# Elody-07/AWR-Adaptive-Weighting-Regression

Hardware: AMD Instinct MI355X
Metric: depth-images/sec (train step) (higher is better)
Workload: dtype f32; 1 GPU; resnet_18-deconv NYU-shape 128x128 J=14 train step (GT-map+fwd+head+Huber+bwd+Adam), batch 64/GPU = BASELINE configs[1]; global_batch=64, img_size=128, joints=14, parallelism=dp1, hipgraph=False, wgrad_streams=2, independent_hw_queues_for_side_streams=3, gemm_products=1, deterministic=False, device_cus=256, nhwc_head_loss=True, launcher=direct

## Files before the change

### awr-adaptive-weighting-regression_amd/csrc/awr_elem.hip

```cpp
#include <math.h>

#include <stdlib.h>

#include "awr_common.h"

namespace awr {

__global__ __launch_bounds__(256) void pack_weight_kernel(const float* __restrict__ w, int d0, int d1, int T, int transpose, int n_pad,
                                                          int ld, float* __restrict__ out) {
    const int64_t total = (int64_t)n_pad * T * ld;
    const int64_t idx = (int64_t)blockIdx.x * 256 + threadIdx.x;
    if (idx >= total) return;
    const int c = (int)(idx % ld);
    const int t = (int)((idx / ld) % T);
    const int n = (int)(idx / ((int64_t)ld * T));
    float v = 0.f;
    if (!transpose) {
        if (n < d0 && c < d1) v = w[((int64_t)n * d1 + c) * T + t];
    } else {
        if (n < d1 && c < d0) v = w[((int64_t)c * d1 + n) * T + t];
    }
    out[idx] = v;
}

__global__ __launch_bounds__(256) void unpack_wgrad_kernel(const float* __restrict__ packed, int d0, int d1, int T, int ld,
                                                           float* __restrict__ grad, int accumulate) {
    const int64_t total = (int64_t)d0 * d1 * T;
    const int64_t idx = (int64_t)blockIdx.x * 256 + threadIdx.x;
    if (idx >= total) return;
    const int t = (int)(idx % T);
    const int b = (int)((idx / T) % d1);
    const int a = (int)(idx / ((int64_t)T * d1));
    const float v = packed[((int64_t)a * T + t) * ld + b];
    grad[idx] = accumulate ? grad[idx] + v : v;
}

template <typename Job>
__device__ __forceinline__ int find_job(const Job* __restrict__ jobs, int n, int64_t idx) {
    int lo = 0, hi = n - 1;
    while (lo < hi) {
        const int mid = (lo + hi + 1) >> 1;
        if (jobs[mid].first <= idx) lo = mid; else hi = mid - 1;
    }
    return lo;
}

__device__ __forceinline__ void store_split_elem(void* split, int64_t idx, float x) {
    const unsigned h = __float_as_uint(x) & 0xFFFF0000u;
    const float r1 = x - __uint_as_float(h);
    const unsigned m = __float_as_uint(r1) & 0xFFFF0000u;
    const unsigned l = __float_as_uint(r1 - __uint_as_float(m));
    unsigned short* o = reinterpret_cast<unsigned short*>(split) + (idx >> 5) * 96 + (idx & 31);
    o[0] = (unsigned short)(h >> 16);
    o[32] = (unsigned short)(m >> 16);
    o[64] = (unsigned short)(l >> 16);
}

constexpr int PACK_TILE = 8192;

__global__ __launch_bounds__(256) void pack_batched_kernel(const awr_pack_job* __restrict__ jobs, int n) {
    __shared__ float tile[PACK_TILE + 64];
    const awr_pack_job jb = jobs[find_job(jobs, n, (int64_t)blockIdx.x)];
    const int r = (int)((int64_t)blockIdx.x - jb.first);
    const int T = jb.T, TS = T | 1, ld = jb.ld;
    const int inner = jb.transpose ? jb.d0 : jb.d1, valid_rows = jb.transpose ? jb.d1 : jb.d0;
    const bool rok = r < valid_rows;
    const int cch = (PACK_TILE / TS) & ~31;
    const int cols = jb.cols > 0 ? jb.cols : ld;
    for (int c0 = 0; c0 < cols; c0 += cch) {
        const int cc = cols - c0 < cch ? cols - c0 : cch;
        for (int i = threadIdx.x; i < cc * T; i += 256) {
            const int c = i / T, t = i - c * T;
            float v = 0.f;
            if (rok && c0 + c < inner)
                v = jb.transpose ? jb.src[((int64_t)(c0 + c) * jb.d1 + r) * T + t] : jb.src[((int64_t)r * jb.d1 + c0 + c) * T + t];
            tile[c * TS + t] = v;
        }
        __syncthreads();
        for (int i = threadIdx.x; i < cc * T; i += 256) {
            const int t = i / cc, c = i - t * cc;
            const float v = tile[c * TS + t];
            const int64_t o = ((int64_t)r * T + t) * ld + c0 + c;
            jb.dst[o] = v;
            if (jb.split) store_split_elem(jb.split, o, v);
        }
        __syncthreads();
    }
}

__global__ __launch_bounds__(256) void split_weight_kernel(const float* __restrict__ packed, void* __restrict__ split, int64_t n) {
    const int64_t idx = (int64_t)blockIdx.x * 256 + threadIdx.x;
    if (idx < n) store_split_elem(split, idx, packed[idx]);
}

__global__ __launch_bounds__(256) void unpack_batched_kernel(const awr_unpack_job* __restrict__ jobs, int n) {
    __shared__ float tile[PACK_TILE + 64];
    const awr_unpack_job jb = jobs[find_job(jobs, n, (int64_t)blockIdx.x)];
    const int a = (int)((int64_t)blockIdx.x - jb.first);
    const int T = jb.T, TS = T | 1, d1 = jb.d1;
    const int cch = (PACK_TILE / TS) & ~31;
    for (int c0 = 0; c0 < d1; c0 += cch) {
        const int cc = d1 - c0 < cch ? d1 - c0 : cch;
        for (int i = threadIdx.x; i < cc * T; i += 256) {
            const int t = i / cc, c = i - t * cc;
            const float* src = jb.packed + ((int64_t)a * T + t) * jb.ld + c0 + c;
            float v = src[0];
            for (int k = 1; k < jb.slots; ++k) v += src[(int64_t)k * jb.slot_stride];
            tile[c * TS + t] = v;
        }
        __syncthreads();
        for (int i = threadIdx.x; i < cc * T; i += 256) {
            const int c = i / T, t = i - c * T;
            jb.grad[((int64_t)a * d1 + c0 + c) * T + t] = tile[c * TS + t];
        }
        __syncthreads();
    }
}

__global__ __launch_bounds__(256) void stem_im2col_kernel(const float* __restrict__ img, int B, int H, int W, float* __restrict__ cols) {
    const int64_t idx = (int64_t)blockIdx.x * 256 + threadIdx.x;
    const int64_t total = (int64_t)B * H * W * 8;
    if (idx >= total) return;
    const int k0 = (int)(idx & 7) * 4;
    const int64_t pix = idx >> 3;
    const int x = (int)(pix % W), y = (int)((pix / W) % H);
    const int64_t b = pix / ((int64_t)W * H);
    float v[4];
#pragma unroll
    for (int i = 0; i < 4; ++i) {
        const int k = k0 + i;
        const int yy = y + k / 5 - 2, xx = x + k % 5 - 2;
        v[i] = (k < 25 && yy >= 0 && yy < H && xx >= 0 && xx < W) ? img[(b * H + yy) * W + xx] : 0.f;
    }
    st4(cols + idx * 4, make_float4(v[0], v[1], v[2], v[3]));
}

__global__ __launch_bounds__(64) void bn_finalize_kernel(double* __restrict__ stats, int C, int nslots, double count, const float* __restrict__ gamma,
                                   const float* __restrict__ beta, float* __restrict__ rmean, float* __restrict__ rvar, float momentum,
                                   float eps, float* __restrict__ scale, float* __restrict__ shift, float* __restrict__ mean_o,
                                   float* __restrict__ invstd_o) {
    const int c = blockIdx.x;
    double s1 = 0.0, s2 = 0.0;
    for (int k = threadIdx.x; k < nslots; k += 64) {
        s1 += stats[(size_t)k * 2 * C + c];
        s2 += stats[(size_t)k * 2 * C + C + c];
        stats[(size_t)k * 2 * C + c] = 0.0;
        stats[(size_t)k * 2 * C + C + c] = 0.0;
    }
    s1 = wave_sum(s1);
    s2 = wave_sum(s2);
    if (threadIdx.x != 0) return;
    const double mean = s1 / count;
    double var = s2 / count - mean * mean;
    if (var < 0.0) var = 0.0;
    const float invstd = (float)(1.0 / sqrt(var + (double)eps));
    const float g = gamma ? gamma[c] : 1.f, b = beta ? beta[c] : 0.f;
    const float sc = g * invstd;
    scale[c] = sc;
    shift[c] = b - (float)mean * sc;
    if (mean_o) mean_o[c] = (float)mean;
    if (invstd_o) invstd_o[c] = invstd;
    if (rmean) rmean[c] = (1.f - momentum) * rmean[c] + momentum * (float)mean;
    if (rvar) {
        const double unb = count > 1.0 ? var * count / (count - 1.0) : var;
        rvar[c] = (1.f - momentum) * rvar[c] + momentum * (float)unb;
    }
}

__global__ void bn_fold_eval_kernel(int C, const float* __restrict__ gamma, const float* __restrict__ beta, const float* __restrict__ rmean,
                                    const float* __restrict__ rvar, float eps, float* __restrict__ scale, float* __restrict__ shift) {
    const int c = blockIdx.x * blockDim.x + threadIdx.x;
    if (c >= C) return;
    const float sc = gamma[c] / sqrtf(rvar[c] + eps);
    scale[c] = sc;
    shift[c] = beta[c] - rmean[c] * sc;
}

struct prod_geom { int H, W, k, s, p, Ho, Wo, in_relu; };
template <int MODE>
__global__ __launch_bounds__(256) void col_reduce_kernel(const float* __restrict__ x, const float* __restrict__ act, const float* __restrict__ y,
                                                         const float* __restrict__ mean, const float* __restrict__ invstd,
                                                         const float* __restrict__ msc, const float* __restrict__ msh, int64_t npix,
                                                         int C, int Cw, int rows_per_block, int nslots, double* __restrict__ out64, float* __restrict__ out32,
                                                         prod_geom pg = prod_geom(), float* __restrict__ pout = nullptr, uint8_t* __restrict__ parg = nullptr) {
    const int cb = blockIdx.y * Cw;
    if (Cw > C - cb) Cw = C - cb;
    const int C4 = Cw >> 2;
    const int rpp = 256 / C4;
    const int cg = threadIdx.x % C4, rg = threadIdx.x / C4;
    const bool active = rg < rpp;
    const int64_t r0 = (int64_t)blockIdx.x * rows_per_block;
    int64_t r1 = r0 + rows_per_block;
    if (r1 > npix) r1 = npix;
    float4 s1 = make_float4(0, 0, 0, 0), s2 = make_float4(0, 0, 0, 0);
    float4 mu = make_float4(0, 0, 0, 0), is = make_float4(1, 1, 1, 1);
    float4 ks = make_float4(0, 0, 0, 0), kt = make_float4(0, 0, 0, 0);
    if (MODE == 1 && active) {
        mu = ld4(mean + cb + cg * 4);
        is = ld4(invstd + cb + cg * 4);
        if (msc) {
            ks = ld4(msc + cb + cg * 4);
            kt = ld4(msh + cb + cg * 4);
        }
    }
    float4 c0 = make_float4(0, 0, 0, 0);
    int nrows = 0;
    if (MODE == 0 && active && r0 + rg < r1) c0 = ld4(x + (r0 + rg) * C + cb + cg * 4);
    auto accum = [&](float4 v, float4 aa, float4 yy) {
        if (MODE == 0) {
            v.x -= c0.x; v.y -= c0.y; v.z -= c0.z; v.w -= c0.w;
            s1.x += v.x; s1.y += v.y; s1.z += v.z; s1.w += v.w;
            s2.x += v.x * v.x; s2.y += v.y * v.y; s2.z += v.z * v.z; s2.w += v.w * v.w;
            ++nrows;
        } else if (MODE == 1) {
            if (act) {
                v.x = aa.x > 0.f ? v.x : 0.f; v.y = aa.y > 0.f ? v.y : 0.f; v.z = aa.z > 0.f ? v.z : 0.f; v.w = aa.w > 0.f ? v.w : 0.f;
            } else if (msc) {
                v.x = yy.x * ks.x + kt.x > 0.f ? v.x : 0.f; v.y = yy.y * ks.y + kt.y > 0.f ? v.y : 0.f;
                v.z = yy.z * ks.z + kt.z > 0.f ? v.z : 0.f; v.w = yy.w * ks.w + kt.w > 0.f ? v.w : 0.f;
            }
            s1.x += v.x; s1.y += v.y; s1.z += v.z; s1.w += v.w;
            s2.x += v.x * ((yy.x - mu.x) * is.x); s2.y += v.y * ((yy.y - mu.y) * is.y);
            s2.z += v.z * ((yy.z - mu.z) * is.z); s2.w += v.w * ((yy.w - mu.w) * is.w);
        } else {
            s1.x += v.x; s1.y += v.y; s1.z += v.z; s1.w += v.w;
        }
    };
    if (MODE >= 3 && active) {
        bool first = true;
        float4 ks4 = make_float4(1, 1, 1, 1), kt4 = make_float4(0, 0, 0, 0);
        if (MODE == 3 && msc) { ks4 = ld4(msc + cb + cg * 4); kt4 = ld4(msh + cb + cg * 4); }
        auto consume = [&](int64_t r, float4 v) {
            st4(pout + r * C + cb + cg * 4, v);
            if (first) { c0 = v; first = false; }
            v.x -= c0.x; v.y -= c0.y; v.z -= c0.z; v.w -= c0.w;
            s1.x += v.x; s1.y += v.y; s1.z += v.z; s1.w += v.w;
            s2.x += v.x * v.x; s2.y += v.y * v.y; s2.z += v.z * v.z; s2.w += v.w * v.w;
            ++nrows;
        };
        int64_t r = r0 + rg;
        constexpr int U = 4;
        if (MODE == 4 || (pg.k == 2 && pg.s == 2 && pg.p == 0)) {
            for (; r + (int64_t)(U - 1) * rpp < r1; r += (int64_t)U * rpp) {
                float4 w[U][4];
                int64_t rr[U];
#pragma unroll
                for (int u = 0; u < U; ++u) {
                    rr[u] = r + (int64_t)u * rpp;
                    const int ox = (int)(rr[u] % pg.Wo), oy = (int)((rr[u] / pg.Wo) % pg.Ho);
                    const int64_t b = rr[u] / ((int64_t)pg.Wo * pg.Ho);
                    if (MODE == 4) {
                        w[u][0] = ld4(x + rr[u] * C + cb + cg * 4);
                        w[u][1] = ld4(act + ((b * pg.H + (oy >> 1)) * pg.W + (ox >> 1)) * C + cb + cg * 4);
                    } else {
                        const float* base = x + ((b * pg.H + 2 * oy) * pg.W + 2 * ox) * C + cb + cg * 4;
                        w[u][0] = ld4(base); w[u][1] = ld4(base + C); w[u][2] = ld4(base + (int64_t)pg.W * C); w[u][3] = ld4(base + (int64_t)pg.W * C + C);
                    }
                }
#pragma unroll
                for (int u = 0; u < U; ++u) {
                    if (MODE == 4) {
                        consume(rr[u], make_float4(w[u][0].x + w[u][1].x, w[u][0].y + w[u][1].y, w[u][0].z + w[u][1].z, w[u][0].w + w[u][1].w));
                    } else {
                        float m[4] = {-INFINITY, -INFINITY, -INFINITY, -INFINITY};
                        int am[4] = {0, 0, 0, 0};
#pragma unroll
                        for (int t = 0; t < 4; ++t) {
                            float4 q = w[u][t];
                            if (msc) {
                                q.x = q.x * ks4.x + kt4.x; q.y = q.y * ks4.y + kt4.y; q.z = q.z * ks4.z + kt4.z; q.w = q.w * ks4.w + kt4.w;
                                if (pg.in_relu) { q.x = fmaxf(q.x, 0.f); q.y = fmaxf(q.y, 0.f); q.z = fmaxf(q.z, 0.f); q.w = fmaxf(q.w, 0.f); }
                            }
                            const float qq[4] = {q.x, q.y, q.z, q.w};
#pragma unroll
                            for (int c = 0; c < 4; ++c)
                                if (qq[c] > m[c]) { m[c] = qq[c]; am[c] = t; }
                        }
                        if (parg) *reinterpret_cast<uchar4*>(parg + rr[u] * C + cb + cg * 4) = make_uchar4((uint8_t)am[0], (uint8_t)am[1], (uint8_t)am[2], (uint8_t)am[3]);
                        consume(rr[u], make_float4(m[0], m[1], m[2], m[3]));
                    }
                }
            }
        }
        for (; r < r1; r += rpp) {
            const int ox = (int)(r % pg.Wo), oy = (int)((r / pg.Wo) % pg.Ho);
            const int64_t b = r / ((int64_t)pg.Wo * pg.Ho);
            float4 v;
            if (MODE == 3) {
                float m[4] = {-INFINITY, -INFINITY, -INFINITY, -INFINITY};
                int am[4] = {0, 0, 0, 0};
                for (int ky = 0; ky < pg.k; ++ky) {
                    const int yy = oy * pg.s - pg.p + ky;
                    if (yy < 0 || yy >= pg.H) continue;
                    for (int kx = 0; kx < pg.k; ++kx) {
                        const int xx = ox * pg.s - pg.p + kx;
                        if (xx < 0 || xx >= pg.W) continue;
                        float4 w = ld4(x + ((b * pg.H + yy) * pg.W + xx) * C + cb + cg * 4);
                        if (msc) {
                            w.x = w.x * ks4.x + kt4.x; w.y = w.y * ks4.y + kt4.y; w.z = w.z * ks4.z + kt4.z; w.w = w.w * ks4.w + kt4.w;
                            if (pg.in_relu) { w.x = fmaxf(w.x, 0.f); w.y = fmaxf(w.y, 0.f); w.z = fmaxf(w.z, 0.f); w.w = fmaxf(w.w, 0.f); }
                        }
                        const float ww[4] = {w.x, w.y, w.z, w.w};
#pragma unroll
                        for (int c = 0; c < 4; ++c)
                            if (ww[c] > m[c]) { m[c] = ww[c]; am[c] = ky * pg.k + kx; }
                    }
                }
                v = make_float4(m[0], m[1], m[2], m[3]);
                if (parg) *reinterpret_cast<uchar4*>(parg + r * C + cb + cg * 4) = make_uchar4((uint8_t)am[0], (uint8_t)am[1], (uint8_t)am[2], (uint8_t)am[3]);
            } else {
                const float4 u = ld4(x + r * C + cb + cg * 4), l = ld4(act + ((b * pg.H + (oy >> 1)) * pg.W + (ox >> 1)) * C + cb + cg * 4);
                v = make_float4(u.x + l.x, u.y + l.y, u.z + l.z, u.w + l.w);
            }
            consume(r, v);
        }
    } else if (active) {
        constexpr int U = 4;
        int64_t r = r0 + rg;
        const float4 z4 = make_float4(0, 0, 0, 0);
        for (; r + (int64_t)(U - 1) * rpp < r1; r += (int64_t)U * rpp) {
            float4 v[U], aa[U], yy[U];
#pragma unroll
            for (int u = 0; u < U; ++u) {
                const int64_t o = (r + (int64_t)u * rpp) * C + cb + cg * 4;
                v[u] = ld4(x + o);
                aa[u] = (MODE == 1 && act) ? ld4(act + o) : z4;
                yy[u] = (MODE == 1) ? ld4(y + o) : z4;
            }
#pragma unroll
            for (int u = 0; u < U; ++u) accum(v[u], aa[u], yy[u]);
        }
        for (; r < r1; r += rpp) {
            const int64_t o = r * C + cb + cg * 4;
            accum(ld4(x + o), (MODE == 1 && act) ? ld4(act + o) : z4, (MODE == 1) ? ld4(y + o) : z4);
        }
    }
    __shared__ double sh1[256][4], sh2[256][4];
    {
        const float p[4] = {s1.x, s1.y, s1.z, s1.w}, q[4] = {s2.x, s2.y, s2.z, s2.w}, c[4] = {c0.x, c0.y, c0.z, c0.w};
#pragma unroll
        for (int k = 0; k < 4; ++k) {
            const double cc = (double)c[k], n = (double)nrows;
            sh1[threadIdx.x][k] = (double)p[k] + n * cc;
            sh2[threadIdx.x][k] = (double)q[k] + 2.0 * cc * (double)p[k] + n * cc * cc;
        }
    }
    __syncthreads();
    if (threadIdx.x < C4) {
        double a[4] = {0, 0, 0, 0}, b[4] = {0, 0, 0, 0};
        for (int g = 0; g < rpp; ++g) {
#pragma unroll
            for (int k = 0; k < 4; ++k) {
                a[k] += sh1[g * C4 + threadIdx.x][k];
                b[k] += sh2[g * C4 + threadIdx.x][k];
            }
        }
#pragma unroll
        for (int k = 0; k < 4; ++k) {
            const int c = cb + threadIdx.x * 4 + k;
            if (MODE == 2) {
                atomicAdd(out32 + c, (float)a[k]);
            } else {
                double* o = out64 + (size_t)(blockIdx.x % nslots) * 2 * C;
                atomicAdd(o + c, a[k]);
                atomicAdd(o + C + c, b[k]);
            }
        }
    }
}

__global__ __launch_bounds__(256) void bn_apply_kernel(const float* __restrict__ x, const float* __restrict__ scale, const float* __restrict__ shift,
                                                       const float* __restrict__ res, int relu, float* __restrict__ out, int64_t n4, int C4) {
    const int64_t i = (int64_t)blockIdx.x * 256 + threadIdx.x;
    if (i >= n4) return;
    const int cg = (int)(i % C4);
    const float4 v = ld4(x + i * 4), sc = ld4(scale + cg * 4), sh = ld4(shift + cg * 4);
    float4 o = make_float4(v.x * sc.x + sh.x, v.y * sc.y + sh.y, v.z * sc.z + sh.z, v.w * sc.w + sh.w);
    if (res) {
        const float4 r = ld4(res + i * 4);
        o.x += r.x; o.y += r.y; o.z += r.z; o.w += r.w;
    }
    if (relu) {
        o.x = fmaxf(o.x, 0.f); o.y = fmaxf(o.y, 0.f); o.z = fmaxf(o.z, 0.f); o.w = fmaxf(o.w, 0.f);
    }
    st4(out + i * 4, o);
}

__global__ __launch_bounds__(64) void bn_bwd_finalize_kernel(double* __restrict__ sums, int C, int nslots, double inv_count, const float* __restrict__ gamma,
                                       const float* __restrict__ invstd, float* __restrict__ coef, float* __restrict__ dgamma,
                                       float* __restrict__ dbeta, int accumulate, const float* __restrict__ mean = nullptr, float* __restrict__ lin = nullptr) {
    const int c = blockIdx.x;
    double s1 = 0.0, s2 = 0.0;
    for (int k = threadIdx.x; k < nslots; k += 64) {
        s1 += sums[(size_t)k * 2 * C + c];
        s2 += sums[(size_t)k * 2 * C + C + c];
        sums[(size_t)k * 2 * C + c] = 0.0;
        sums[(size_t)k * 2 * C + C + c] = 0.0;
    }
    s1 = wave_sum(s1);
    s2 = wave_sum(s2);
    if (threadIdx.x != 0) return;
    coef[c] = (float)(s1 * inv_count);
    coef[C + c] = (float)(s2 * inv_count);
    coef[2 * C + c] = (gamma ? gamma[c] : 1.f) * invstd[c];
    if (dgamma) dgamma[c] = (accumulate ? dgamma[c] : 0.f) + (float)s2;
    if (dbeta) dbeta[c] = (accumulate ? dbeta[c] : 0.f) + (float)s1;
    if (lin) {
        const float gi = coef[2 * C + c];
        lin[c] = gi;
        lin[C + c] = -(gi * invstd[c]) * coef[C + c];
        lin[2 * C + c] = -gi * coef[c];
        lin[3 * C + c] = mean[c];
    }
}

__global__ __launch_bounds__(256) void bn_bwd_apply_kernel(const float* dout, const float* __restrict__ act, const float* __restrict__ y,
                                                           const float* __restrict__ mean, const float* __restrict__ invstd,
                                                           const float* __restrict__ msc, const float* __restrict__ msh,
                                                           const float* __restrict__ coef, int64_t n4, int C, float* dy, const float* dy_add,
                                                           float* __restrict__ g_out) {
    const int C4 = C >> 2;
    const int64_t i = (int64_t)blockIdx.x * 256 + threadIdx.x;
    if (i >= n4) return;
    const int cg = (int)(i % C4);
    float4 g = ld4(dout + i * 4);
    const float4 yy = ld4(y + i * 4), mu = ld4(mean + cg * 4), is = ld4(invstd + cg * 4);
    if (act) {
        const float4 a = ld4(act + i * 4);
        g.x = a.x > 0.f ? g.x : 0.f; g.y = a.y > 0.f ? g.y : 0.f; g.z = a.z > 0.f ? g.z : 0.f; g.w = a.w > 0.f ? g.w : 0.f;
    } else if (msc) {
        const float4 ks = ld4(msc + cg * 4), kt = ld4(msh + cg * 4);
        g.x = yy.x * ks.x + kt.x > 0.f ? g.x : 0.f; g.y = yy.y * ks.y + kt.y > 0.f ? g.y : 0.f;
        g.z = yy.z * ks.z + kt.z > 0.f ? g.z : 0.f; g.w = yy.w * ks.w + kt.w > 0.f ? g.w : 0.f;
    }
    if (g_out) st4(g_out + i * 4, g);
    const float4 k1 = ld4(coef + cg * 4), k2 = ld4(coef + C + cg * 4), gi = ld4(coef + 2 * C + cg * 4);
    float4 o;
    o.x = gi.x * (g.x - k1.x - (yy.x - mu.x) * is.x * k2.x);
    o.y = gi.y * (g.y - k1.y - (yy.y - mu.y) * is.y * k2.y);
    o.z = gi.z * (g.z - k1.z - (yy.z - mu.z) * is.z * k2.z);
    o.w = gi.w * (g.w - k1.w - (yy.w - mu.w) * is.w * k2.w);
    if (dy_add) {
        const float4 e = ld4(dy_add + i * 4);
        o.x += e.x; o.y += e.y; o.z += e.z; o.w += e.w;
    }
    st4(dy + i * 4, o);
}

__global__ __launch_bounds__(256) void relu_bwd_kernel(const float* __restrict__ dout, const float* __restrict__ act, float* __restrict__ g, int64_t n4) {
    const int64_t i = (int64_t)blockIdx.x * 256 + threadIdx.x;
    if (i >= n4) return;
    float4 v = ld4(dout + i * 4);
    const float4 a = ld4(act + i * 4);
    v.x = a.x > 0.f ? v.x : 0.f; v.y = a.y > 0.f ? v.y : 0.f; v.z = a.z > 0.f ? v.z : 0.f; v.w = a.w > 0.f ? v.w : 0.f;
    st4(g + i * 4, v);
}

__global__ __launch_bounds__(256) void add_kernel(const float* __restrict__ a, const float* __restrict__ b, float* __restrict__ out, int64_t n4) {
    const int64_t i = (int64_t)blockIdx.x * 256 + threadIdx.x;
    if (i >= n4) return;
    const float4 x = ld4(a + i * 4), y = ld4(b + i * 4);
    st4(out + i * 4, make_float4(x.x + y.x, x.y + y.y, x.z + y.z, x.w + y.w));
}

__global__ __launch_bounds__(256) void maxpool_fwd_kernel(const float* __restrict__ x, const float* __restrict__ isc, const float* __restrict__ ish,
                                                          int in_relu, int B, int H, int W, int C, int k, int s, int p, int Ho, int Wo,
                                                          float* __restrict__ out, uint8_t* __restrict__ arg) {
    const int C4 = C >> 2;
    const int64_t i = (int64_t)blockIdx.x * 256 + threadIdx.x;
    const int64_t total = (int64_t)B * Ho * Wo * C4;
    if (i >= total) return;
    const int cg = (int)(i % C4);
    const int64_t pix = i / C4;
    const int ox = (int)(pix % Wo), oy = (int)((pix / Wo) % Ho);
    const int64_t b = pix / ((int64_t)Wo * Ho);
    float m[4] = {-INFINITY, -INFINITY, -INFINITY, -INFINITY};
    int a[4] = {0, 0, 0, 0};
    float4 sc = make_float4(1, 1, 1, 1), sh = make_float4(0, 0, 0, 0);
    if (isc) {
        sc = ld4(isc + cg * 4);
        sh = ld4(ish + cg * 4);
    }
    for (int ky = 0; ky < k; ++ky) {
        const int yy = oy * s - p + ky;
        if (yy < 0 || yy >= H) continue;
        for (int kx = 0; kx < k; ++kx) {
            const int xx = ox * s - p + kx;
            if (xx < 0 || xx >= W) continue;
            float4 v = ld4(x + ((b * H + yy) * W + xx) * C + cg * 4);
            if (isc) {
                v.x = v.x * sc.x + sh.x; v.y = v.y * sc.y + sh.y; v.z = v.z * sc.z + sh.z; v.w = v.w * sc.w + sh.w;
                if (in_relu) { v.x = fmaxf(v.x, 0.f); v.y = fmaxf(v.y, 0.f); v.z = fmaxf(v.z, 0.f); v.w = fmaxf(v.w, 0.f); }
            }
            const float vv[4] = {v.x, v.y, v.z, v.w};
#pragma unroll
            for (int c = 0; c < 4; ++c)
                if (vv[c] > m[c]) {
                    m[c] = vv[c];
                    a[c] = ky * k + kx;
                }
        }
    }
    st4(out + i * 4, make_float4(m[0], m[1], m[2], m[3]));
    if (arg) *reinterpret_cast<uchar4*>(arg + i * 4) = make_uchar4((uint8_t)a[0], (uint8_t)a[1], (uint8_t)a[2], (uint8_t)a[3]);
}

__global__ __launch_bounds__(256) void maxpool_bwd_kernel(const float* __restrict__ dout, const uint8_t* __restrict__ arg, int B, int H, int W,
                                                          int C, int k, int s, int p, int Ho, int Wo, float* __restrict__ dx, int accumulate) {
    const int C4 = C >> 2;
    const int64_t i = (int64_t)blockIdx.x * 256 + threadIdx.x;
    const int64_t total = (int64_t)B * H * W * C4;
    if (i >= total) return;
    const int cg = (int)(i % C4);
    const int64_t pix = i / C4;
    const int x = (int)(pix % W), y = (int)((pix / W) % H);
    const int64_t b = pix / ((int64_t)W * H);
    float acc[4] = {0, 0, 0, 0};
    int oy0 = (y + p - k + 1 + s - 1) / s;
    if (y + p - k + 1 < 0) oy0 = 0;
    int ox0 = (x + p - k + 1 + s - 1) / s;
    if (x + p - k + 1 < 0) ox0 = 0;
    const int oy1 = min((y + p) / s, Ho - 1), ox1 = min((x + p) / s, Wo - 1);
    for (int oy = oy0; oy <= oy1; ++oy)
        for (int ox = ox0; ox <= ox1; ++ox) {
            const int local = (y - (oy * s - p)) * k + (x - (ox * s - p));
            const int64_t o = (((b * Ho + oy) * Wo + ox) * C4 + cg) * 4;
            const uchar4 a = *reinterpret_cast<const uchar4*>(arg + o);
            const float4 d = ld4(dout + o);
            if (a.x == local) acc[0] += d.x;
            if (a.y == local) acc[1] += d.y;
            if (a.z == local) acc[2] += d.z;
            if (a.w == local) acc[3] += d.w;
        }
    if (accumulate) {
        const float4 e = ld4(dx + i * 4);
        acc[0] += e.x; acc[1] += e.y; acc[2] += e.z; acc[3] += e.w;
    }
    st4(dx + i * 4, make_float4(acc[0], acc[1], acc[2], acc[3]));
}

__global__ __launch_bounds__(256) void upsample2_add_kernel(const float* __restrict__ up1, const float* __restrict__ low, int B, int Hl, int Wl, int C,
                                                            float* __restrict__ out) {
    const int C4 = C >> 2;
    const int H = Hl * 2, W = Wl * 2;
    const int64_t i = (int64_t)blockIdx.x * 256 + threadIdx.x;
    const int64_t total = (int64_t)B * H * W * C4;
    if (i >= total) return;
    const int cg = (int)(i % C4);
    const int64_t pix = i / C4;
    const int x = (int)(pix % W), y = (int)((pix / W) % H);
    const int64_t b = pix / ((int64_t)W * H);
    const float4 u = ld4(up1 + i * 4), l = ld4(low + (((b * Hl + (y >> 1)) * Wl + (x >> 1)) * C4 + cg) * 4);
    st4(out + i * 4, make_float4(u.x + l.x, u.y + l.y, u.z + l.z, u.w + l.w));
}

__global__ __launch_bounds__(256) void upsample2_bwd_kernel(const float* __restrict__ dout, int B, int Hl, int Wl, int C, float* __restrict__ dlow,
                                                            int accumulate) {
    const int C4 = C >> 2;
    const int H = Hl * 2, W = Wl * 2;
    const int64_t i = (int64_t)blockIdx.x * 256 + threadIdx.x;
    const int64_t total = (int64_t)B * Hl * Wl * C4;
    if (i >= total) return;
    const int cg = (int)(i % C4);
    const int64_t pix = i / C4;
    const int x = (int)(pix % Wl), y = (int)((pix / Wl) % Hl);
    const int64_t b = pix / ((int64_t)Wl * Hl);
    float4 s = make_float4(0, 0, 0, 0);
#pragma unroll
    for (int dy = 0; dy < 2; ++dy)
#pragma unroll
        for (int dx = 0; dx < 2; ++dx) {
            const float4 d = ld4(dout + (((b * H + 2 * y + dy) * W + 2 * x + dx) * C4 + cg) * 4);
            s.x += d.x; s.y += d.y; s.z += d.z; s.w += d.w;
        }
    if (accumulate) {
        const float4 e = ld4(dlow + i * 4);
        s.x += e.x; s.y += e.y; s.z += e.z; s.w += e.w;
    }
    st4(dlow + i * 4, s);
}

__global__ __launch_bounds__(256) void nhwc_to_nchw_kernel(const float* __restrict__ in, int P, int Cp, int C, float* __restrict__ out) {
    __shared__ float tile[32][33];
    const int b = blockIdx.z, p0 = blockIdx.x * 32, c0 = blockIdx.y * 32;
    const int tx = threadIdx.x & 31, ty = threadIdx.x >> 5;
    for (int r = ty; r < 32; r += 8) {
        const int p = p0 + r, c = c0 + tx;
        tile[r][tx] = (p < P && c < Cp) ? in[((int64_t)b * P + p) * Cp + c] : 0.f;
    }
    __syncthreads();
    for (int r = ty; r < 32; r += 8) {
        const int c = c0 + r, p = p0 + tx;
        if (c < C && p < P) out[((int64_t)b * C + c) * P + p] = tile[tx][r];
    }
}

__global__ __launch_bounds__(256) void nchw_to_nhwc_kernel(const float* __restrict__ in, int P, int Cp, int C, float* __restrict__ out) {
    __shared__ float tile[32][33];
    const int b = blockIdx.z, p0 = blockIdx.x * 32, c0 = blockIdx.y * 32;
    const int tx = threadIdx.x & 31, ty = threadIdx.x >> 5;
    for (int r = ty; r < 32; r += 8) {
        const int c = c0 + r, p = p0 + tx;
        tile[r][tx] = (c < C && p < P) ? in[((int64_t)b * C + c) * P + p] : 0.f;
    }
    __syncthreads();
    for (int r = ty; r < 32; r += 8) {
        const int p = p0 + r, c = c0 + tx;
        if (p < P && c < Cp) out[((int64_t)b * P + p) * Cp + c] = tile[tx][r];
    }
}

static inline unsigned nblk(int64_t n) { return (unsigned)((n + 255) / 256); }

static int col_reduce_launch(int mode, const float* x, const float* act, const float* y, const float* mean, const float* invstd,
                             const float* msc, const float* msh, int64_t npix, int C, double* out64, float* out32, int nslots, hipStream_t st,
                             prod_geom pg = prod_geom(), float* pout = nullptr, uint8_t* parg = nullptr) {
    AWR_REQUIRE(C % 4 == 0 && C >= 4 && (C <= 1024 || C % 1024 == 0), "channel reduction: C=%d must be a multiple of 4 up to 1024, or a multiple of 1024", C);
    AWR_REQUIRE(npix > 0 && nslots >= 0, "channel reduction: empty tensor");
    if (nslots == 0) nslots = AWR_STAT_SLOTS;
    const int Cw = C <= 1024 ? C : 1024;
    const unsigned nchunk = (unsigned)(C / Cw);
    const int rpp = 256 / (Cw / 4);
    int64_t rows = (npix + AWR_REDUCE_MAX_BLOCKS - 1) / AWR_REDUCE_MAX_BLOCKS;
    if (rows < 64) rows = 64;
    rows = (rows + rpp - 1) / rpp * rpp;
    const unsigned grid = (unsigned)((npix + rows - 1) / rows);
    if (mode == 0)
        hipLaunchKernelGGL(col_reduce_kernel<0>, dim3(grid, nchunk), dim3(256), 0, st, x, act, y, mean, invstd, msc, msh, npix, C, Cw, (int)rows, nslots, out64, out32);
    else if (mode == 1)
        hipLaunchKernelGGL(col_reduce_kernel<1>, dim3(grid, nchunk), dim3(256), 0, st, x, act, y, mean, invstd, msc, msh, npix, C, Cw, (int)rows, nslots, out64, out32);
    else if (mode == 3)
        hipLaunchKernelGGL(col_reduce_kernel<3>, dim3(grid, nchunk), dim3(256), 0, st, x, act, y, mean, invstd, msc, msh, npix, C, Cw, (int)rows, nslots, out64, out32, pg, pout, parg);
    else if (mode == 4)
        hipLaunchKernelGGL(col_reduce_kernel<4>, dim3(grid, nchunk), dim3(256), 0, st, x, act, y, mean, invstd, msc, msh, npix, C, Cw, (int)rows, nslots, out64, out32, pg, pout, parg);
    else
        hipLaunchKernelGGL(col_reduce_kernel<2>, dim3(grid, nchunk), dim3(256), 0, st, x, act, y, mean, invstd, msc, msh, npix, C, Cw, (int)rows, nslots, out64, out32);
    return check_launch("col_reduce_kernel");
}

static int g_deterministic = []() { const char* e = getenv("AWR_DETERMINISTIC"); return e ? atoi(e) != 0 : 0; }();

}

using namespace awr;

extern "C" {

int awr_pack_weight(const float* w, int d0, int d1, int T, int transpose, int n_pad, int ld, float* packed, void* stream) {
    AWR_REQUIRE(w && packed && d0 > 0 && d1 > 0 && T > 0, "pack_weight: bad arguments");
    const int rows = transpose ? d1 : d0, inner = transpose ? d0 : d1;
    AWR_REQUIRE(n_pad >= rows && ld >= inner, "pack_weight: n_pad=%d < %d or ld=%d < %d", n_pad, rows, ld, inner);
    hipLaunchKernelGGL(pack_weight_kernel, dim3(nblk((int64_t)n_pad * T * ld)), dim3(256), 0, as_stream(stream), w, d0, d1, T, transpose, n_pad,
                       ld, packed);
    return check_launch("pack_weight_kernel");
}

#ifdef AWR_STUDY
__global__ __launch_bounds__(256) void split_act_kernel(const float* __restrict__ x, const float* __restrict__ scale, const float* __restrict__ shift, int relu,
                                                        int64_t n8, int C, char* __restrict__ split) {
    const int64_t i = (int64_t)blockIdx.x * 256 + threadIdx.x;
    if (i >= n8) return;
    const int64_t e = i * 8;
    float v[8];
    *reinterpret_cast<float4*>(v) = ld4(x + e);
    *reinterpret_cast<float4*>(v + 4) = ld4(x + e + 4);
    if (scale) {
        const int c = (int)(e % C);
        float sc[8], sh[8];
        *reinterpret_cast<float4*>(sc) = ld4(scale + c); *reinterpret_cast<float4*>(sc + 4) = ld4(scale + c + 4);
        *reinterpret_cast<float4*>(sh) = ld4(shift + c); *reinterpret_cast<float4*>(sh + 4) = ld4(shift + c + 4);
#pragma unroll
        for (int k = 0; k < 8; ++k) v[k] = v[k] * sc[k] + sh[k];
    }
    if (relu) {
#pragma unroll
        for (int k = 0; k < 8; ++k) v[k] = fmaxf(v[k], 0.f);
    }
    unsigned h[8], m[8], l[8];
#pragma unroll
    for (int k = 0; k < 8; ++k) {
        h[k] = __float_as_uint(v[k]) & 0xFFFF0000u;
        const float r1 = v[k] - __uint_as_float(h[k]);
        m[k] = __float_as_uint(r1) & 0xFFFF0000u;
        l[k] = __float_as_uint(r1 - __uint_as_float(m[k]));
    }
    auto pk = [](unsigned lo, unsigned hi) { return (lo >> 16) | (hi & 0xFFFF0000u); };
    char* dst = split + (e >> 5) * 192 + (e & 31) * 2;
    *reinterpret_cast<uint4*>(dst) = make_uint4(pk(h[0], h[1]), pk(h[2], h[3]), pk(h[4], h[5]), pk(h[6], h[7]));
    *reinterpret_cast<uint4*>(dst + 64) = make_uint4(pk(m[0], m[1]), pk(m[2], m[3]), pk(m[4], m[5]), pk(m[6], m[7]));
    *reinterpret_cast<uint4*>(dst + 128) = make_uint4(pk(l[0], l[1]), pk(l[2], l[3]), pk(l[4], l[5]), pk(l[6], l[7]));
}

int awr_split_act(const float* x, const float* scale, const float* shift, int relu, int64_t npix, int C, void* split, void* stream) {
    AWR_REQUIRE(x && split && npix > 0 && C > 0 && C % 32 == 0 && (scale == nullptr) == (shift == nullptr), "split_act: C must be a positive multiple of 32");
    const int64_t n8 = npix * C / 8;
    hipLaunchKernelGGL(split_act_kernel, dim3(nblk(n8)), dim3(256), 0, as_stream(stream), x, scale, shift, relu, n8, C, static_cast<char*>(split));
    return check_launch("split_act_kernel");
}
#endif

int awr_split_weight(const float* packed, void* split, int64_t n, void* stream) {
    AWR_REQUIRE(packed && split && n > 0 && n % 32 == 0, "split_weight: n must be a positive multiple of 32");
    hipLaunchKernelGGL(split_weight_kernel, dim3(nblk(n)), dim3(256), 0, as_stream(stream), packed, split, n);
    return check_launch("split_weight_kernel");
}

int awr_unpack_wgrad(const float* packed, int d0, int d1, int T, int ld, float* grad, int accumulate, void* stream) {
    AWR_REQUIRE(packed && grad && d0 > 0 && d1 > 0 && T > 0 && ld >= d1, "unpack_wgrad: bad arguments");
    hipLaunchKernelGGL(unpack_wgrad_kernel, dim3(nblk((int64_t)d0 * d1 * T)), dim3(256), 0, as_stream(stream), packed, d0, d1, T, ld, grad,
                       accumulate);
    return check_launch("unpack_wgrad_kernel");
}

int awr_pack_weights_batched(const awr_pack_job* jobs_dev, int njobs, int64_t total_rows, void* stream) {
    AWR_REQUIRE(jobs_dev && njobs > 0 && total_rows > 0 && total_rows < (1LL << 31), "pack_weights_batched: bad arguments");
    hipLaunchKernelGGL(pack_batched_kernel, dim3((unsigned)total_rows), dim3(256), 0, as_stream(stream), jobs_dev, njobs);
    return check_launch("pack_batched_kernel");
}

int awr_unpack_wgrads_batched(const awr_unpack_job* jobs_dev, int njobs, int64_t total_rows, void* stream) {
    AWR_REQUIRE(jobs_dev && njobs > 0 && total_rows > 0 && total_rows < (1LL << 31), "unpack_wgrads_batched: bad arguments");
    hipLaunchKernelGGL(unpack_batched_kernel, dim3((unsigned)total_rows), dim3(256), 0, as_stream(stream), jobs_dev, njobs);
    return check_launch("unpack_batched_kernel");
}

int awr_stem_im2col(const float* img, int B, int H, int W, float* cols, void* stream) {
    AWR_REQUIRE(img && cols && B > 0 && H > 0 && W > 0, "stem_im2col: bad arguments");
    hipLaunchKernelGGL(stem_im2col_kernel, dim3(nblk((int64_t)B * H * W * 8)), dim3(256), 0, as_stream(stream), img, B, H, W, cols);
    return check_launch("stem_im2col_kernel");
}

int awr_set_deterministic(int on) {
    g_deterministic = on != 0;
    return AWR_OK;
}

int awr_get_deterministic(void) { return g_deterministic; }

int awr_bn_finalize(double* stats, int C, int64_t count, const float* gamma, const float* beta, float* running_mean, float* running_var,
                    float momentum, float eps, float* scale, float* shift, float* mean, float* invstd, int nslots, void* stream) {
    AWR_REQUIRE(stats && scale && shift && C > 0 && count > 0 && nslots >= 0, "bn_finalize: bad arguments");
    hipLaunchKernelGGL(bn_finalize_kernel, dim3(C), dim3(64), 0, as_stream(stream), stats, C, nslots ? nslots : AWR_STAT_SLOTS, (double)count, gamma, beta,
                       running_mean, running_var, momentum, eps, scale, shift, mean, invstd);
    return check_launch("bn_finalize_kernel");
}

int awr_bn_fold_eval(int C, const float* gamma, const float* beta, const float* running_mean, const float* running_var, float eps,
                     float* scale, float* shift, void* stream) {
    AWR_REQUIRE(gamma && beta && running_mean && running_var && scale && shift && C > 0, "bn_fold_eval: bad arguments");
    hipLaunchKernelGGL(bn_fold_eval_kernel, dim3((C + 127) / 128), dim3(128), 0, as_stream(stream), C, gamma, beta, running_mean, running_var,
                       eps, scale, shift);
    return check_launch("bn_fold_eval_kernel");
}

int awr_channel_stats(const float* x, int64_t npix, int C, double* stats, int nslots, void* stream) {
    AWR_REQUIRE(x && stats, "channel_stats: null pointer");
    return col_reduce_launch(0, x, nullptr, nullptr, nullptr, nullptr, nullptr, nullptr, npix, C, stats, nullptr, nslots, as_stream(stream));
}

int awr_bn_apply(const float* x, const float* scale, const float* shift, const float* res, int relu, float* out, int64_t npix, int C,
                 void* stream) {
    AWR_REQUIRE(x && scale && shift && out && npix > 0 && C % 4 == 0, "bn_apply: bad arguments");
    const int64_t n4 = npix * (C / 4);
    hipLaunchKernelGGL(bn_apply_kernel, dim3(nblk(n4)), dim3(256), 0, as_stream(stream), x, scale, shift, res, relu, out, n4, C / 4);
    return check_launch("bn_apply_kernel");
}

int awr_bn_bwd_reduce(const float* dout, const float* act, const float* y, const float* mean, const float* invstd, const float* mask_scale,
                      const float* mask_shift, int64_t npix, int C, double* sums, int nslots, void* stream) {
    AWR_REQUIRE(dout && y && mean && invstd && sums, "bn_bwd_reduce: null pointer");
    AWR_REQUIRE((mask_scale == nullptr) == (mask_shift == nullptr) && !(act && mask_scale), "bn_bwd_reduce: give act OR mask_scale+mask_shift");
    return col_reduce_launch(1, dout, act, y, mean, invstd, mask_scale, mask_shift, npix, C, sums, nullptr, nslots, as_stream(stream));
}

int awr_bn_bwd_apply(const float* dout, const float* act, const float* y, const float* mean, const float* invstd, const float* gamma,
                     const float* mask_scale, const float* mask_shift, double* sums, float* coef, int64_t npix, int C, float* dy,
                     const float* dy_add, float* g_out, float* dgamma, float* dbeta, int accumulate, int nslots, void* stream) {
    AWR_REQUIRE(dout && y && mean && invstd && sums && coef && dy && npix > 0 && C % 4 == 0 && nslots >= 0, "bn_bwd_apply: bad arguments");
    hipLaunchKernelGGL(bn_bwd_finalize_kernel, dim3(C), dim3(64), 0, as_stream(stream), sums, C, nslots ? nslots : AWR_STAT_SLOTS, 1.0 / (double)npix, gamma,
                       invstd, coef, dgamma, dbeta, accumulate);
    if (int e = check_launch("bn_bwd_finalize_kernel")) return e;
    const int64_t n4 = npix * (C / 4);
#ifdef AWR_STUDY_HOOKS
    static const bool exp_skip = getenv("AWR_EXP_NO_BN_BWD_APPLY") != nullptr;
    if (exp_skip) return AWR_OK;
#endif
    hipLaunchKernelGGL(bn_bwd_apply_kernel, dim3(nblk(n4)), dim3(256), 0, as_stream(stream), dout, act, y, mean, invstd, mask_scale, mask_shift,
                       coef, n4, C, dy, dy_add, g_out);
    return check_launch("bn_bwd_apply_kernel");
}

int awr_bn_bwd_finalize(double* sums, int C, int64_t count, const float* gamma, const float* invstd, float* coef, float* dgamma, float* dbeta,
                        int accumulate, int nslots, void* stream) {
    AWR_REQUIRE(sums && invstd && coef && C > 0 && count > 0 && nslots >= 0, "bn_bwd_finalize: bad arguments");
    hipLaunchKernelGGL(bn_bwd_finalize_kernel, dim3(C), dim3(64), 0, as_stream(stream), sums, C, nslots ? nslots : AWR_STAT_SLOTS, 1.0 / (double)count, gamma,
                       invstd, coef, dgamma, dbeta, accumulate);
    return check_launch("bn_bwd_finalize_kernel");
}

int awr_bn_bwd_finalize_lin(double* sums, int C, int64_t count, const float* gamma, const float* mean, const float* invstd, float* coef, float* lin4,
                            float* dgamma, float* dbeta, int accumulate, int nslots, void* stream) {
    AWR_REQUIRE(sums && mean && invstd && coef && lin4 && C > 0 && count > 0 && nslots >= 0, "bn_bwd_finalize_lin: bad arguments");
    hipLaunchKernelGGL(bn_bwd_finalize_kernel, dim3(C), dim3(64), 0, as_stream(stream), sums, C, nslots ? nslots : AWR_STAT_SLOTS, 1.0 / (double)count, gamma,
                       invstd, coef, dgamma, dbeta, accumulate, mean, lin4);
    return check_launch("bn_bwd_finalize_kernel");
}

int awr_bn_bwd_apply_only(const float* dout, const float* act, const float* y, const float* mean, const float* invstd, const float* mask_scale,
                          const float* mask_shift, const float* coef, int64_t npix, int C, float* dy, const float* dy_add, float* g_out, void* stream) {
    AWR_REQUIRE(dout && y && mean && invstd && coef && dy && npix > 0 && C % 4 == 0, "bn_bwd_apply_only: bad arguments");
    const int64_t n4 = npix * (C / 4);
    hipLaunchKernelGGL(bn_bwd_apply_kernel, dim3(nblk(n4)), dim3(256), 0, as_stream(stream), dout, act, y, mean, invstd, mask_scale, mask_shift,
                       coef, n4, C, dy, dy_add, g_out);
    return check_launch("bn_bwd_apply_kernel");
}

int awr_relu_bwd(const float* dout, const float* act, float* g, int64_t n, void* stream) {
    AWR_REQUIRE(dout && act && g && n > 0 && n % 4 == 0, "relu_bwd: bad arguments");
    hipLaunchKernelGGL(relu_bwd_kernel, dim3(nblk(n / 4)), dim3(256), 0, as_stream(stream), dout, act, g, n / 4);
    return check_launch("relu_bwd_kernel");
}

int awr_add(const float* a, const float* b, float* out, int64_t n, void* stream) {
    AWR_REQUIRE(a && b && out && n > 0 && n % 4 == 0, "add: bad arguments");
    hipLaunchKernelGGL(add_kernel, dim3(nblk(n / 4)), dim3(256), 0, as_stream(stream), a, b, out, n / 4);
    return check_launch("add_kernel");
}

int awr_bias_grad(const float* dy, int64_t npix, int C, float* db, int accumulate, void* stream) {
    AWR_REQUIRE(dy && db, "bias_grad: null pointer");
    AWR_REQUIRE(C % 4 == 0 && C >= 4 && (C <= 1024 || C % 1024 == 0) && npix > 0, "bias_grad: C=%d must be a multiple of 4 up to 1024, or a multiple of 1024, and npix > 0", C);
    if (!accumulate && hipMemsetAsync(db, 0, sizeof(float) * C, as_stream(stream)) != hipSuccess) {
        set_error("bias_grad: hipMemsetAsync failed");
        return AWR_ERR_HIP;
    }
    return col_reduce_launch(2, dy, nullptr, nullptr, nullptr, nullptr, nullptr, nullptr, npix, C, nullptr, db, 0, as_stream(stream));
}

int awr_maxpool_fwd(const float* x, const float* in_scale, const float* in_shift, int in_relu, int B, int H, int W, int C, int k, int s, int p,
                    float* out, uint8_t* argmax, void* stream) {
    AWR_REQUIRE((in_scale == nullptr) == (in_shift == nullptr), "maxpool_fwd: in_scale/in_shift must come together");
    AWR_REQUIRE(x && out && B > 0 && C % 4 == 0 && k >= 1 && k <= 15 && s >= 1 && p >= 0 && p < k, "maxpool_fwd: bad arguments");
    const int Ho = (H + 2 * p - k) / s + 1, Wo = (W + 2 * p - k) / s + 1;
    hipLaunchKernelGGL(maxpool_fwd_kernel, dim3(nblk((int64_t)B * Ho * Wo * (C / 4))), dim3(256), 0, as_stream(stream), x, in_scale, in_shift, in_relu, B, H, W,
                       C, k, s, p, Ho, Wo, out, argmax);
    return check_launch("maxpool_fwd_kernel");
}

int awr_maxpool_fwd_stats(const float* x, const float* in_scale, const float* in_shift, int in_relu, int B, int H, int W, int C, int k, int s, int p,
                          float* out, uint8_t* argmax, double* stats, int nslots, void* stream) {
    AWR_REQUIRE((in_scale == nullptr) == (in_shift == nullptr), "maxpool_fwd_stats: in_scale/in_shift must come together");
    AWR_REQUIRE(x && out && stats && B > 0 && k >= 1 && k <= 15 && s >= 1 && p >= 0 && p < k, "maxpool_fwd_stats: bad arguments");
    prod_geom pg;
    pg.H = H; pg.W = W; pg.k = k; pg.s = s; pg.p = p; pg.Ho = (H + 2 * p - k) / s + 1; pg.Wo = (W + 2 * p - k) / s + 1; pg.in_relu = in_relu;
    return col_reduce_launch(3, x, nullptr, nullptr, nullptr, nullptr, in_scale, in_shift, (int64_t)B * pg.Ho * pg.Wo, C, stats, nullptr, nslots, as_stream(stream),
                             pg, out, argmax);
}

int awr_upsample2_add_stats(const float* up1, const float* low, int B, int Hl, int Wl, int C, float* out, double* stats, int nslots, void* stream) {
    AWR_REQUIRE(up1 && low && out && stats && B > 0, "upsample2_add_stats: bad arguments");
    prod_geom pg;
    pg.H = Hl; pg.W = Wl; pg.k = 0; pg.s = 0; pg.p = 0; pg.Ho = 2 * Hl; pg.Wo = 2 * Wl; pg.in_relu = 0;
    return col_reduce_launch(4, up1, low, nullptr, nullptr, nullptr, nullptr, nullptr, (int64_t)B * pg.Ho * pg.Wo, C, stats, nullptr, nslots, as_stream(stream),
                             pg, out, nullptr);
}

int awr_maxpool_bwd(const float* dout, const uint8_t* argmax, int B, int H, int W, int C, int k, int s, int p, float* dx, int accumulate,
                    void* stream) {
    AWR_REQUIRE(dout && argmax && dx && B > 0 && C % 4 == 0 && k >= 1 && s >= 1, "maxpool_bwd: bad arguments");
    const int Ho = (H + 2 * p - k) / s + 1, Wo = (W + 2 * p - k) / s + 1;
    hipLaunchKernelGGL(maxpool_bwd_kernel, dim3(nblk((int64_t)B * H * W * (C / 4))), dim3(256), 0, as_stream(stream), dout, argmax, B, H, W, C,
                       k, s, p, Ho, Wo, dx, accumulate);
    return check_launch("maxpool_bwd_kernel");
}

int awr_upsample2_add(const float* up1, const float* low, int B, int Hl, int Wl, int C, float* out, void* stream) {
    AWR_REQUIRE(up1 && low && out && B > 0 && C % 4 == 0, "upsample2_add: bad arguments");
    hipLaunchKernelGGL(upsample2_add_kernel, dim3(nblk((int64_t)B * Hl * Wl * C)), dim3(256), 0, as_stream(stream), up1, low, B, Hl, Wl, C, out);
    return check_launch("upsample2_add_kernel");
}

int awr_upsample2_bwd(const float* dout, int B, int Hl, int Wl, int C, float* dlow, int accumulate, void* stream) {
    AWR_REQUIRE(dout && dlow && B > 0 && C % 4 == 0, "upsample2_bwd: bad arguments");
    hipLaunchKernelGGL(upsample2_bwd_kernel, dim3(nblk((int64_t)B * Hl * Wl * (C / 4))), dim3(256), 0, as_stream(stream), dout, B, Hl, Wl, C, dlow, accumulate);
    return check_launch("upsample2_bwd_kernel");
}

int awr_nhwc_to_nchw(const float* in, int B, int P, int Cp, int C, float* out, void* stream) {
    AWR_REQUIRE(in && out && B > 0 && P > 0 && C > 0 && Cp >= C, "nhwc_to_nchw: bad arguments");
    hipLaunchKernelGGL(nhwc_to_nchw_kernel, dim3((P + 31) / 32, (C + 31) / 32, B), dim3(256), 0, as_stream(stream), in, P, Cp, C, out);
    return check_launch("nhwc_to_nchw_kernel");
}

int awr_nchw_to_nhwc(const float* in, int B, int P, int Cp, int C, float* out, void* stream) {
    AWR_REQUIRE(in && out && B > 0 && P > 0 && C > 0 && Cp >= C, "nchw_to_nhwc: bad arguments");
    hipLaunchKernelGGL(nchw_to_nhwc_kernel, dim3((P + 31) / 32, (Cp + 31) / 32, B), dim3(256), 0, as_stream(stream), in, P, Cp, C, out);
    return check_launch("nchw_to_nhwc_kernel");
}

}
```

Before: 4932 images/s.

## Vectorize and coalesce batched weight pack/unpack kernels with wave-ballot job lookup

Rewrites the batched weight pack and wgrad unpack kernels so global loads and stores go through aligned float4 accesses with alignment-aware slot iteration. For transposed packs, several rows are grouped into one tile so short lines are read contiguously, and the LDS tile is halved. Job lookup now uses two wave-wide ballots instead of a serial binary search. These changes target uncoalesced, strided scalar traffic in the per-step weight repack and gradient reduction, in exchange for more complex indexing that carries edge-case correctness risk.

```diff
diff --git a/awr-adaptive-weighting-regression_amd/csrc/awr_elem.hip b/awr-adaptive-weighting-regression_amd/csrc/awr_elem.hip
--- a/awr-adaptive-weighting-regression_amd/csrc/awr_elem.hip
+++ b/awr-adaptive-weighting-regression_amd/csrc/awr_elem.hip
@@ -37,6 +37,16 @@
 
 template <typename Job>
 __device__ __forceinline__ int find_job(const Job* __restrict__ jobs, int n, int64_t idx) {
+    if (n <= 4096) {
+        const int lane = threadIdx.x & 63, step = (n + 63) >> 6;
+        const int a = lane * step;
+        int blk = __popcll(__ballot(a < n && jobs[a < n ? a : 0].first <= idx)) - 1;
+        if (blk < 0) blk = 0;
+        const int b = blk * step + lane;
+        const bool in = lane < step && b < n;
+        const int k = __popcll(__ballot(in && jobs[in ? b : 0].first <= idx));
+        return blk * step + (k > 0 ? k - 1 : 0);
+    }
     int lo = 0, hi = n - 1;
     while (lo < hi) {
         const int mid = (lo + hi + 1) >> 1;
@@ -56,34 +66,158 @@
     o[64] = (unsigned short)(l >> 16);
 }
 
-constexpr int PACK_TILE = 8192;
-
-__global__ __launch_bounds__(256) void pack_batched_kernel(const awr_pack_job* __restrict__ jobs, int n) {
+constexpr int PACK_THREADS = 256;
+
+#define AWR_GLOBAL __attribute__((address_space(1)))
+typedef float f32x4 __attribute__((ext_vector_type(4)));
+__device__ __forceinline__ float gld(const float* p) { return *(const AWR_GLOBAL float*)p; }
+__device__ __forceinline__ void gst(float* p, float v) { *(AWR_GLOBAL float*)p = v; }
+__device__ __forceinline__ float4 gld4(const float* p) {
+    const f32x4 v = *(const AWR_GLOBAL f32x4*)p;
+    return make_float4(v.x, v.y, v.z, v.w);
+}
+__device__ __forceinline__ void gst4(float* p, float4 v) {
+    const f32x4 w = {v.x, v.y, v.z, v.w};
+    *(AWR_GLOBAL f32x4*)p = w;
+}
+
+template <typename F>
+__device__ __forceinline__ void for_line_slots(const float* p, int nl, int n, int64_t pitch, bool wide, F&& f) {
+    const bool vec = wide && (nl == 1 || (pitch & 3) == 0);
+    const int mis = vec ? (int)((reinterpret_cast<uintptr_t>(p) >> 2) & 3) : 0;
+    const int S = vec ? (mis + n + 3) >> 2 : n;
+    const int total = nl * S;
+    int i = threadIdx.x;
+    if (i >= total) return;
+    int line = i / S, s = i - line * S;
+    const int dl = PACK_THREADS / S, ds = PACK_THREADS - dl * S;
+    for (; i < total; i += PACK_THREADS) {
+        if (vec) {
+            const int e0 = 4 * s - mis;
+            if (e0 >= 0 && e0 + 4 <= n) {
+                f(line, e0, true);
+            } else {
+#pragma unroll
+                for (int k = 0; k < 4; ++k)
+                    if (e0 + k >= 0 && e0 + k < n) f(line, e0 + k, false);
+            }
+        } else {
+            f(line, s, false);
+        }
+        line += dl;
+        s += ds;
+        if (s >= S) { s -= S; ++line; }
+    }
+}
+
+template <typename F>
+__device__ __forceinline__ void for_span_slots(const float* p, int n, int T, F&& f) {
+    const int mis = (int)((reinterpret_cast<uintptr_t>(p) >> 2) & 3);
+    const int S = (mis + n + 3) >> 2;
+    int s = threadIdx.x;
+    if (s >= S) return;
+    const int v0 = 4 * s - mis + 4 * T;
+    int c = v0 / T - 4, t = v0 % T;
+    const int dc = 4 * PACK_THREADS / T, dt = 4 * PACK_THREADS - dc * T;
+    for (; s < S; s += PACK_THREADS) {
+        const int e0 = 4 * s - mis;
+        if (e0 >= 0 && e0 + 4 <= n) {
+            f(e0, c, t, true);
+        } else {
+            int cc = c, tt = t;
+#pragma unroll
+            for (int k = 0; k < 4; ++k) {
+                if (e0 + k >= 0 && e0 + k < n) f(e0 + k, cc, tt, false);
+                if (++tt == T) { tt = 0; ++cc; }
+            }
+        }
+        c += dc;
+        t += dt;
+        if (t >= T) { t -= T; ++c; }
+    }
+}
+
+constexpr int PACK_TILE = 4096;
+
+__device__ __forceinline__ int chunk_cols(int P) {
+    const int cw = PACK_TILE / P;
+    return cw >= 32 ? cw & ~31 : cw;
+}
+
+__global__ __launch_bounds__(PACK_THREADS) void pack_batched_kernel(const awr_pack_job* __restrict__ jobs, int n) {
     __shared__ float tile[PACK_TILE + 64];
     const awr_pack_job jb = jobs[find_job(jobs, n, (int64_t)blockIdx.x)];
     const int r = (int)((int64_t)blockIdx.x - jb.first);
-    const int T = jb.T, TS = T | 1, ld = jb.ld;
-    const int inner = jb.transpose ? jb.d0 : jb.d1, valid_rows = jb.transpose ? jb.d1 : jb.d0;
-    const bool rok = r < valid_rows;
-    const int cch = (PACK_TILE / TS) & ~31;
+    const int T = jb.T, ld = jb.ld, d1 = jb.d1;
+    const bool tr = jb.transpose != 0;
+    const int inner = tr ? jb.d0 : d1, valid_rows = tr ? d1 : jb.d0;
     const int cols = jb.cols > 0 ? jb.cols : ld;
-    for (int c0 = 0; c0 < cols; c0 += cch) {
-        const int cc = cols - c0 < cch ? cols - c0 : cch;
-        for (int i = threadIdx.x; i < cc * T; i += 256) {
-            const int c = i / T, t = i - c * T;
-            float v = 0.f;
-            if (rok && c0 + c < inner)
-                v = jb.transpose ? jb.src[((int64_t)(c0 + c) * jb.d1 + r) * T + t] : jb.src[((int64_t)r * jb.d1 + c0 + c) * T + t];
-            tile[c * TS + t] = v;
+    int R = 1;
+    if (tr)
+        while (R < 32 && 2 * R * T <= 100) R *= 2;
+    const int r0 = r & ~(R - 1), part = r - r0;
+    const int Rn = jb.rows - r0 < R ? jb.rows - r0 : R;
+    const int Lq = Rn * T, P = Lq | 1;
+    const int vr = valid_rows - r0 < 0 ? 0 : (valid_rows - r0 < Rn ? valid_rows - r0 : Rn);
+    const int Lv = vr * T;
+    int cw = chunk_cols(P);
+    if (Rn > 1) {
+        const int want = ((cols + Rn - 1) / Rn + 31) & ~31;
+        if (want < cw) cw = want;
+    }
+    for (int c0 = part * cw; c0 < cols; c0 += Rn * cw) {
+        const int cc = cols - c0 < cw ? cols - c0 : cw;
+        const int cv = inner - c0 < 0 ? 0 : (inner - c0 < cc ? inner - c0 : cc);
+        if (cv > 0 && Lv > 0) {
+            if (tr) {
+                const int64_t pitch = (int64_t)d1 * T;
+                const float* src = jb.src + ((int64_t)c0 * d1 + r0) * T;
+                for_line_slots(src, cv, Lv, pitch, true, [&](int c, int q, bool four) {
+                    float* o = tile + c * P + q;
+                    if (four) {
+                        const float4 v = gld4(src + c * pitch + q);
+                        o[0] = v.x; o[1] = v.y; o[2] = v.z; o[3] = v.w;
+                    } else {
+                        o[0] = gld(src + c * pitch + q);
+                    }
+                });
+            } else {
+                const float* src = jb.src + ((int64_t)r * d1 + c0) * T;
+                for_span_slots(src, cv * T, T, [&](int e, int c, int t, bool four) {
+                    if (four) {
+                        const float4 v = gld4(src + e);
+                        const float x[4] = {v.x, v.y, v.z, v.w};
+#pragma unroll
+                        for (int k = 0; k < 4; ++k) {
+                            tile[c * P + t] = x[k];
+                            if (++t == T) { t = 0; ++c; }
+                        }
+                    } else {
+                        tile[c * P + t] = gld(src + e);
+                    }
+                });
+            }
         }
         __syncthreads();
-        for (int i = threadIdx.x; i < cc * T; i += 256) {
-            const int t = i / cc, c = i - t * cc;
-            const float v = tile[c * TS + t];
-            const int64_t o = ((int64_t)r * T + t) * ld + c0 + c;
-            jb.dst[o] = v;
-            if (jb.split) store_split_elem(jb.split, o, v);
-        }
+        const int64_t obase = (int64_t)r0 * T * ld + c0;
+        for_line_slots(jb.dst + obase, Lq, cc, ld, true, [&](int q, int c, bool four) {
+            const int64_t o = obase + (int64_t)q * ld + c;
+            const bool qok = q < Lv;
+            if (four) {
+                float x[4];
+#pragma unroll
+                for (int k = 0; k < 4; ++k) x[k] = qok && c + k < cv ? tile[(c + k) * P + q] : 0.f;
+                gst4(jb.dst + o, make_float4(x[0], x[1], x[2], x[3]));
+                if (jb.split) {
+#pragma unroll
+                    for (int k = 0; k < 4; ++k) store_split_elem(jb.split, o + k, x[k]);
+                }
+            } else {
+                const float v = qok && c < cv ? tile[c * P + q] : 0.f;
+                gst(jb.dst + o, v);
+                if (jb.split) store_split_elem(jb.split, o, v);
+            }
+        });
         __syncthreads();
     }
 }
@@ -93,26 +227,48 @@
     if (idx < n) store_split_elem(split, idx, packed[idx]);
 }
 
-__global__ __launch_bounds__(256) void unpack_batched_kernel(const awr_unpack_job* __restrict__ jobs, int n) {
+__global__ __launch_bounds__(PACK_THREADS) void unpack_batched_kernel(const awr_unpack_job* __restrict__ jobs, int n) {
     __shared__ float tile[PACK_TILE + 64];
     const awr_unpack_job jb = jobs[find_job(jobs, n, (int64_t)blockIdx.x)];
     const int a = (int)((int64_t)blockIdx.x - jb.first);
-    const int T = jb.T, TS = T | 1, d1 = jb.d1;
-    const int cch = (PACK_TILE / TS) & ~31;
-    for (int c0 = 0; c0 < d1; c0 += cch) {
-        const int cc = d1 - c0 < cch ? d1 - c0 : cch;
-        for (int i = threadIdx.x; i < cc * T; i += 256) {
-            const int t = i / cc, c = i - t * cc;
-            const float* src = jb.packed + ((int64_t)a * T + t) * jb.ld + c0 + c;
-            float v = src[0];
-            for (int k = 1; k < jb.slots; ++k) v += src[(int64_t)k * jb.slot_stride];
-            tile[c * TS + t] = v;
-        }
+    const int T = jb.T, P = T | 1, d1 = jb.d1, ld = jb.ld, slots = jb.slots;
+    const int64_t stride = jb.slot_stride;
+    const bool wide = slots <= 1 || (stride & 3) == 0;
+    const int cw = chunk_cols(P);
+    for (int c0 = 0; c0 < d1; c0 += cw) {
+        const int cc = d1 - c0 < cw ? d1 - c0 : cw;
+        const float* src = jb.packed + (int64_t)a * T * ld + c0;
+        for_line_slots(src, T, cc, ld, wide, [&](int t, int c, bool four) {
+            const float* s = src + (int64_t)t * ld + c;
+            float* o = tile + c * P + t;
+            if (four) {
+                float4 v = gld4(s);
+                for (int k = 1; k < slots; ++k) {
+                    const float4 w = gld4(s + k * stride);
+                    v.x += w.x; v.y += w.y; v.z += w.z; v.w += w.w;
+                }
+                o[0] = v.x; o[P] = v.y; o[2 * P] = v.z; o[3 * P] = v.w;
+            } else {
+                float v = gld(s);
+                for (int k = 1; k < slots; ++k) v += gld(s + k * stride);
+                o[0] = v;
+            }
+        });
         __syncthreads();
-        for (int i = threadIdx.x; i < cc * T; i += 256) {
-            const int c = i / T, t = i - c * T;
-            jb.grad[((int64_t)a * d1 + c0 + c) * T + t] = tile[c * TS + t];
-        }
+        float* dst = jb.grad + ((int64_t)a * d1 + c0) * T;
+        for_span_slots(dst, cc * T, T, [&](int e, int c, int t, bool four) {
+            if (four) {
+                float x[4];
+#pragma unroll
+                for (int k = 0; k < 4; ++k) {
+                    x[k] = tile[c * P + t];
+                    if (++t == T) { t = 0; ++c; }
+                }
+                gst4(dst + e, make_float4(x[0], x[1], x[2], x[3]));
+            } else {
+                gst(dst + e, tile[c * P + t]);
+            }
+        });
         __syncthreads();
     }
 }
@@ -714,13 +870,13 @@
 
 int awr_pack_weights_batched(const awr_pack_job* jobs_dev, int njobs, int64_t total_rows, void* stream) {
     AWR_REQUIRE(jobs_dev && njobs > 0 && total_rows > 0 && total_rows < (1LL << 31), "pack_weights_batched: bad arguments");
-    hipLaunchKernelGGL(pack_batched_kernel, dim3((unsigned)total_rows), dim3(256), 0, as_stream(stream), jobs_dev, njobs);
+    hipLaunchKernelGGL(pack_batched_kernel, dim3((unsigned)total_rows), dim3(PACK_THREADS), 0, as_stream(stream), jobs_dev, njobs);
     return check_launch("pack_batched_kernel");
 }
 
 int awr_unpack_wgrads_batched(const awr_unpack_job* jobs_dev, int njobs, int64_t total_rows, void* stream) {
     AWR_REQUIRE(jobs_dev && njobs > 0 && total_rows > 0 && total_rows < (1LL << 31), "unpack_wgrads_batched: bad arguments");
-    hipLaunchKernelGGL(unpack_batched_kernel, dim3((unsigned)total_rows), dim3(256), 0, as_stream(stream), jobs_dev, njobs);
+    hipLaunchKernelGGL(unpack_batched_kernel, dim3((unsigned)total_rows), dim3(PACK_THREADS), 0, as_stream(stream), jobs_dev, njobs);
     return check_launch("unpack_batched_kernel");
 }
 
```

New measurement: 4968 images/s (median of 6 runs). Within noise of the previous version (+0.7%).
